# sdrobert/pydrobert-pytorch

Measured on AMD Instinct MI355X. Metric: utterances/sec (N=4096,T=512) error_rate+ctc_beam at 1/2/4/8 GPU, higher is better.
Workload: dtype f32

## Files before the change

### pydrobert-pytorch_amd/csrc/ctc_frame.hpp

```cpp
#pragma once
#include "wave_select.hpp"

namespace pdt {

#ifdef PDT_STAMPS
__device__ unsigned long long g_stamps[16];
__device__ unsigned long long *g_stamp_lds_dummy;
#define PDT_STAMP(ph)                                                        \
  do {                                                                       \
    const unsigned long long now_ = __builtin_readcyclecounter();           \
    pdt_stamp_acc[ph] += (unsigned)(now_ - stamp_last_);                     \
    stamp_last_ = now_;                                                      \
  } while (0)
#define PDT_STAMP_BEGIN unsigned long long stamp_last_ = __builtin_readcyclecounter()
#else
#define PDT_STAMP(ph) do {} while (0)
#define PDT_STAMP_BEGIN do {} while (0)
#endif

#ifdef PDT_STATS
__device__ unsigned long long g_stats[24];
#define PDT_STAT(i) do { if (lane_id() == 0) atomicAdd(&g_stats[i], 1ull); } while (0)
#else
#define PDT_STAT(i) do {} while (0)
#endif

#ifdef PDT_UTT_STATS
__device__ unsigned g_utt_stats[8192 * 4];
#define PDT_UTT(k, v) do { pdt_utt_acc[k] += (unsigned)(v); } while (0)
#else
#define PDT_UTT(k, v) do {} while (0)
#endif

constexpr int kMaxWidth = 32;

struct CtcArgs {
  const float *logits;
  int64_t lg_st, lg_sn, lg_sv;
  const int64_t *lens;
  int T, N, V, W, S;
  int64_t *y;
  int64_t *y_lens;
  float *y_probs;
  int2 *trie;
  int2 *ckpt;
  unsigned char *grow;
  int ckpt_shift, ckpt_count;
  int lds_per_wave, waves_per_wg;
  int exact_div;
  int no_lean_extra;
  int no_steady;
};

struct Beam {
  float nb, b;
  int last, len, node;
  unsigned isp;
  int origin = 0;
};

__device__ __forceinline__ u64 readlane_u64(u64 v, int l) {
  const unsigned lo = (unsigned)__builtin_amdgcn_readlane((int)(unsigned)v, l);
  const unsigned hi = (unsigned)__builtin_amdgcn_readlane((int)(unsigned)(v >> 32), l);
  return ((u64)hi << 32) | lo;
}
__device__ __forceinline__ float readlane_f(float v, int l) {
  return __int_as_float(__builtin_amdgcn_readlane(__float_as_int(v), l));
}
__device__ __forceinline__ float shfl_f(float v, int l) { return __int_as_float(shfl_i(__float_as_int(v), l)); }
__device__ __forceinline__ unsigned fresh_zero() {
  unsigned z;
  asm volatile("v_mov_b32 %0, 0" : "=v"(z));
  return z;
}

struct DenseCtx {
  const float *ext;
  int64_t ext_sk, ext_sv;
  const int64_t *y_prev;
  int64_t yp_ss, yp_sk;
  int S;
  int lists_ready;
  const float *etab = nullptr;
  int etab_stride = 0;
  const int16_t *y_prev16 = nullptr;
  const int *slot = nullptr;
  const int *list_id = nullptr;
  unsigned closed = 0u;
  const int *lpos = nullptr;
  int lpos_stride = 0;
};

__host__ __device__ inline int nxt_stride(int W) { return W * W < 128 ? 128 : W * W; }
__host__ __device__ inline int consumer_scratch_bytes(int W) {
  return (2 * nxt_stride(W) * 4 + (W > 0 ? W : 1) * 4 * 3 + 7) & ~7;
}

struct FrameLds {
  u64 *surv;
  int *tl_tok;
  float *tl_p;
  unsigned char *pos;
  unsigned *chm;
  int *info;
  int *nxt_old, *nxt_new;
  int list_len;
  float *hdr;
  int2 *trie_u = nullptr;
  float pl_in = 0.0f, pblank_in = 0.0f;
  static __host__ __device__ size_t bytes(int V, int W, int Kp, bool dense) {
    const int RS = W > Kp ? W : Kp;
    size_t b = (size_t)PDT_SURV_CAP * 8 + (size_t)(dense ? Kp : 1) * PDT_WAVE * 8;
    b += dense ? 0 : (size_t)((V + 15) & ~15);
    b += (size_t)RS * 4 + (size_t)2 * W * 4 + (dense ? 0 : (size_t)2 * W * W * 4);
    return (b + 15) & ~(size_t)15;
  }
  __device__ void carve(unsigned char *base, int V, int W, int Kp, bool dense) {
    const int RS = W > Kp ? W : Kp, L = dense ? Kp : 1;
    surv = reinterpret_cast<u64 *>(base);
    tl_tok = reinterpret_cast<int *>(surv + PDT_SURV_CAP);
    tl_p = reinterpret_cast<float *>(tl_tok + L * PDT_WAVE);
    chm = reinterpret_cast<unsigned *>(tl_p + L * PDT_WAVE);
    info = reinterpret_cast<int *>(chm + RS);
    nxt_old = info + 2 * W;
    nxt_new = nxt_old + (dense ? 0 : W * W);
    pos = reinterpret_cast<unsigned char *>(nxt_new + (dense ? 0 : W * W));
  }
};

__device__ __forceinline__ int ctc_list_len(int V, int W, int Kp) {
  const int K = min(W, Kp * (V + 1));
  return min(V, K + Kp);
}

template <bool LONG = false>
__device__ __forceinline__ void build_shared_list(const float *p, float inv, int V, int M, u64 *surv,
                                                  int *tl_tok, float *tl_p, unsigned char *pos,
                                                  const unsigned *lmax_in = nullptr,
                                                  unsigned *probe = nullptr, int probe_rank = 1) {
  const int lane = lane_id();
  const u64 tk = wave_top_sorted<LONG, true>(p, V, M, surv, lmax_in, probe, probe_rank);
  if (lane < M) {
    const int tok = (int)idx_of(tk);
    tl_tok[lane] = tok;
    tl_p[lane] = p[tok] * inv;
    pos[tok] = (unsigned char)lane;
  }
}

#if defined(PDT_STAMPS)
#define PDT_STAMP_PARAM , unsigned *pdt_stamp_acc
#define PDT_STAMP_ARG , pdt_stamp_acc
#elif defined(PDT_UTT_STATS)
#define PDT_STAMP_PARAM , unsigned *pdt_utt_acc
#define PDT_STAMP_ARG , pdt_utt_acc
#else
#define PDT_STAMP_PARAM
#define PDT_STAMP_ARG
#endif

template <bool DENSE, bool ROWLESS = false, bool TRIE = !DENSE>
__device__ __forceinline__ bool ctc_frame(Beam &bm, const float *p, const float inv, const int V,
                                          const int W, const int Kp, const int t,
                                          const int64_t n, const CtcArgs &a, const DenseCtx &dc,
                                          const FrameLds &L, int &new_src, int &new_tok,
                                          int &new_kind PDT_STAMP_PARAM) {
  int lane = lane_id();
  asm volatile("" : "+v"(lane));
  const bool live = lane < Kp;
  const int K = min(W, Kp * (V + 1));
  const int M = min(V, K + Kp);
  const int me = live ? lane : 0;
  PDT_STAMP_BEGIN;

  if (DENSE && !dc.lists_ready) {
    for (int k = 0; k < Kp; ++k) {
      const u64 tk = wave_top_sorted_strided<true>(dc.ext + k * dc.ext_sk, dc.ext_sv, V, M, L.surv);
      if (lane < M) {
        L.tl_tok[k * PDT_WAVE + lane] = (int)idx_of(tk);
        L.tl_p[k * PDT_WAVE + lane] = fkey_inv(key_of(tk));
      }
      wave_sync();
    }
  }
  PDT_STAMP(1);
  auto list_of = [&](const int k) -> int { return DENSE ? (dc.list_id ? dc.list_id[k] : k) : 0; };
  const int my_list = list_of(me);
  const int *mt = L.tl_tok + my_list * PDT_WAVE;

  static_assert(!(DENSE && ROWLESS), "the row-less form reads the shared list");
  const float p_blank = ROWLESS ? L.pblank_in : p[V] * inv;
  const int lastc = min(max(bm.last, 0), V - 1);
  const float pl = ROWLESS ? L.pl_in : p[lastc] * inv;
  const float e_last = DENSE ? (dc.etab ? dc.etab[my_list * dc.etab_stride + me] : dc.ext[me * dc.ext_sk + lastc * dc.ext_sv]) : pl;
  const float tot = bm.nb + bm.b;
  const float B = tot * p_blank;
  float NB = bm.nb * pl;
  const bool valid_beam = live && tot > -PDT_INF;
  wave_sync();

  const int c_list = (DENSE || ROWLESS) ? M : min(L.list_len, M);
  const bool full_list = DENSE || ROWLESS || c_list >= M;
  int jl = -1;
  u64 avail = 0ull;
  bool s1_open = valid_beam, s2_open = valid_beam;
// ... 472 lines not shown
  PDT_STAMP(3);
  const int srcl = new_kind >= 0 ? new_src : lane;
  float NB_s = NB, B_s = B;
  int last_s = lastc, len_s = bm.len, node_s = bm.node;
  unsigned isp_s = bm.isp;
  if (!steady_f) {
    NB_s = shfl_f(NB, srcl), B_s = shfl_f(B, srcl);
    last_s = shfl_i(lastc, srcl), len_s = shfl_i(bm.len, srcl), node_s = shfl_i(bm.node, srcl);
    isp_s = (unsigned)shfl_i((int)bm.isp, srcl);
  }
  const bool is_ext = new_kind == 0 || new_kind == 1;
  const bool is_valid = new_kind >= 0;
  Beam nw;
  nw.nb = !is_valid ? -PDT_INF : (is_ext ? new_mass : NB_s);
  nw.b = !is_valid ? -PDT_INF : (is_ext ? 0.0f : B_s);
  nw.last = !is_valid ? 0 : (is_ext ? new_tok : last_s);
  nw.len = !is_valid ? 0 : len_s + (is_ext ? 1 : 0);
  nw.node = !is_valid ? -1 : (is_ext ? t * W + lane : node_s);
  if (TRIE) nw.origin = steady_f ? bm.origin : shfl_i(bm.origin, srcl);
  if (TRIE && is_valid && is_ext)
    *reinterpret_cast<int2 *>(reinterpret_cast<char *>(L.trie_u) + (unsigned)(t * W + lane) * 8u) = make_int2(node_s, new_tok);

  PDT_STAMP(4);
  const int RS = W > Kp ? W : Kp;
  if (!steady_f) {
    if (lane < RS) L.chm[lane] = fresh_zero();
    wave_sync();
    if (is_valid) atomicOr(&L.chm[new_src], 1u << lane);
  }
  if (is_valid) {
    L.info[2 * lane] = new_tok;
    L.info[2 * lane + 1] = len_s | (new_src << 20) | ((is_ext ? 1 : 0) << 28);
  }
  wave_sync();
  PDT_STAMP(10);
  unsigned isp_new = 0u;
  bool need_walk = false;
  bool pairs_done = false;
#ifndef PDT_NO_PAIR_PREFIX
#ifndef PDT_PAIR_DENSE
#define PDT_PAIR_DENSE 8
#endif
  if (__builtin_expect(TRIE && W <= 16 && !a.no_lean_extra && __ballot(is_valid && __popc(isp_s) > PDT_PAIR_DENSE) != 0ull, 0)) {
    const int pa = lane & 15, pq = lane >> 4;
    const u64 vmask = __ballot(is_valid);
    const int a_tok = shfl_i(new_tok, pa);
    const int a_w = shfl_i(len_s | (new_src << 20) | ((is_ext ? 1 : 0) << 28) | ((is_valid ? 1 : 0) << 29), pa);
    const unsigned a_isp = (unsigned)shfl_i((int)isp_s, pa);
    const int a_len_s = a_w & 0xFFFFF, a_src = (a_w >> 20) & 0xFF;
    const bool a_ext = (a_w >> 28) & 1, a_valid = (a_w >> 29) & 1;
    const int a_len = a_len_s + (a_ext ? 1 : 0);
    unsigned bits = 0u, walks = 0u;
#pragma unroll
    for (int r = 0; r < 4; ++r) {
      const int b = 4 * r + pq;
      const int tok_b = L.info[2 * b], w1 = L.info[2 * b + 1];
      const int lenB = w1 & 0xFFFFF, src_b = (w1 >> 20) & 0xFF;
      const bool ext_b = (w1 >> 28) & 1;
      const int len_b = lenB + (ext_b ? 1 : 0);
      bool pref = a_valid && ((vmask >> b) & 1ull) && b != pa && ((a_isp >> src_b) & 1u) && !(a_len > len_b);
      int tok_at = -1;
      if (pref) tok_at = lenB > a_len_s ? L.nxt_old[a_src * W + src_b] : (ext_b ? tok_b : -1);
      pref = pref && !(a_ext && tok_at != a_tok);
      bool walk = false;
      if (pref && a_len < len_b) {
        int nx;
        if (!a_ext) {
          nx = tok_at;
        } else if (lenB == a_len_s + 1) {
          nx = tok_b;
        } else {
          nx = -(2 + b);
          walk = true;
        }
        L.nxt_new[pa * W + b] = nx;
      }
      const u64 m = __ballot(pref), wm = __ballot(walk);
      const unsigned lo = (unsigned)m >> pa, hi = (unsigned)(m >> 32) >> pa;
      bits |= ((lo & 1u) | ((lo >> 15) & 2u) | ((hi & 1u) << 2) | ((hi >> 13) & 8u)) << (4 * r);
      walks |= (unsigned)(wm | (wm >> 16) | (wm >> 32) | (wm >> 48));
    }
    if (is_valid) {
      isp_new = bits | (1u << lane);
      need_walk = (walks >> lane) & 1u;
    }
    pairs_done = true;
    wave_sync();
  }
#endif
  if (is_valid && !pairs_done) {
    unsigned cand = 0u;
    if (steady_f) cand = isp_s;
    else
      for (unsigned m = isp_s; m; m &= m - 1u) cand |= L.chm[__builtin_ctz(m)];
    cand &= ~(1u << lane);
    isp_new = 1u << lane;
    while (cand) {
      const int b = __builtin_ctz(cand);
      cand &= cand - 1u;
      const int tok_b = L.info[2 * b], w1 = L.info[2 * b + 1];
      const int lenB = w1 & 0xFFFFF, src_b = (w1 >> 20) & 0xFF;
      const bool ext_b = (w1 >> 28) & 1;
      const int len_b = lenB + (ext_b ? 1 : 0);
      if (nw.len > len_b) continue;
      int tok_at;
      if (lenB > len_s)
        tok_at = !TRIE ? (dc.y_prev16 ? (int)dc.y_prev16[(int64_t)len_s * dc.yp_ss + (dc.slot ? dc.slot[src_b] : src_b) * dc.yp_sk]
                                      : (int)dc.y_prev[(int64_t)len_s * dc.yp_ss + (dc.slot ? dc.slot[src_b] : src_b) * dc.yp_sk])
                       : L.nxt_old[new_src * W + src_b];
      else
        tok_at = ext_b ? tok_b : -1;
      if (is_ext && tok_at != new_tok) continue;
      isp_new |= 1u << b;
      if (TRIE && nw.len < len_b) {
        int nx;
        if (!is_ext) {
          nx = tok_at;
        } else if (lenB == len_s + 1) {
          nx = tok_b;
        } else {
          nx = -(2 + b);
          need_walk = true;
        }
        L.nxt_new[lane * W + b] = nx;
      }
    }
  }
  if (TRIE && __ballot(need_walk)) {
    __builtin_amdgcn_fence(__ATOMIC_RELEASE, "agent");
    for (int b = 0; b < K; ++b) {
      const int node_b = __builtin_amdgcn_readlane(node_s, b);
      const int lenB = __builtin_amdgcn_readlane(len_s, b);
      if (need_walk && ((isp_new >> b) & 1u) && L.nxt_new[lane * W + b] == -(2 + b)) {
        int node = node_b, depth = lenB, tok = -1;
        while (node >= 0) {
          const int2 *rec = a.trie + ((int64_t)n * a.T * W + node);
          const int par_ = __hip_atomic_load(&rec->x, __ATOMIC_RELAXED, __HIP_MEMORY_SCOPE_AGENT);
          tok = __hip_atomic_load(&rec->y, __ATOMIC_RELAXED, __HIP_MEMORY_SCOPE_AGENT);
          if (depth == nw.len + 1) break;
          node = par_;
          --depth;
        }
        L.nxt_new[lane * W + b] = tok;
      }
    }
  }
  nw.isp = isp_new;
  bm = nw;
  wave_sync();
  PDT_STAMP(5);
  return list_sufficed;
}

template <int JW = 4>
__device__ __forceinline__ void walk_trie_segments(const int2 *tab, const int nseg, const int W, const int2 *trie_u,
                                                   int64_t *y_n, const int64_t row_stride) {
  const int lane = lane_id();
  for (int base = 0; base < nseg; base += JW * PDT_WAVE) {
    int node[JW], ps[JW], stop[JW], col[JW];
#pragma unroll
    for (int j = 0; j < JW; ++j) {
      const int sg = base + j * PDT_WAVE + lane;
      node[j] = -1, ps[j] = -1, stop[j] = 0, col[j] = 0;
      if (sg < nseg) {
        const int c = sg / W;
        col[j] = sg - c * W;
        const int2 top = tab[sg];
        stop[j] = c > 0 ? tab[sg - W].y : 0;
        node[j] = top.x;
        ps[j] = top.y - 1;
      }
    }
    bool any = true;
    while (any) {
      any = false;
      u64 rec[JW];
      bool act[JW];
#pragma unroll
      for (int j = 0; j < JW; ++j) {
        act[j] = ps[j] >= stop[j] && node[j] >= 0;
        rec[j] = 0ull;
        if (act[j]) rec[j] = *reinterpret_cast<const u64 *>(trie_u + node[j]);
      }
#pragma unroll
      for (int j = 0; j < JW; ++j) {
        if (act[j]) {
          y_n[(int64_t)ps[j] * row_stride + col[j]] = (int64_t)(int)(unsigned)(rec[j] >> 32);
          node[j] = (int)(unsigned)rec[j];
          --ps[j];
          any = true;
        }
      }
    }
  }
}

}
```

### pydrobert-pytorch_amd/csrc/ctc_search.hip

```cpp
#include "ctc_ring.hpp"
#include "switches.hpp"

#include <cstdlib>

namespace pdt {

template <int P, int NT = -1, bool INREG = (P == 1), bool GROW = false, int WC = -1, int VC = -1, bool PAIR = false>
__global__ void __launch_bounds__(256, INREG ? 8 : 4)
ctc_search_kernel(const CtcArgs a, const RingLayout rl_arg) {
  static_assert(!INREG || P == 1, "the register-resident row pass is a one-producer form");
  static_assert((WC > 0 && VC > 0) ? (P == 1 && INREG && !GROW) : true, "compile-time shapes: the register-resident form");
  const RingLayout rl = (WC > 0 && VC > 0) ? ring_layout(VC, WC, PDT_RING_STAGES, PDT_UTT_PER_WG, 1) : rl_arg;
  static_assert(!GROW || !INREG, "rows in the workspace are a form of the generic row pass");
  static_assert(NT < 0 || INREG, "compile-time chunk counts belong to the register-resident row pass");
  extern __shared__ __align__(16) unsigned char smem[];
  const int lane = lane_id();
  const int wave = __builtin_amdgcn_readfirstlane((int)(threadIdx.x >> 6));
  const int u = wave / (P + 1);
  const int role = wave - u * (P + 1);
  const bool producer = role < P;
  const int64_t n_raw = (int64_t)xcd_remap(blockIdx.x, gridDim.x) * rl.utt_per_wg + u;
  const bool idle = u >= rl.utt_per_wg || n_raw >= a.N;
  const int64_t n = idle ? 0 : n_raw;
  const int V = VC > 0 ? VC : a.V, W = WC > 0 ? WC : a.W;
// ... 299 lines not shown
#pragma unroll
          for (int i = 0; i < kPrefetch; ++i) {
            if (i > nt) break;
            if (i < nt) {
              pre[i] = nrow[(int64_t)(i * PDT_WAVE) * lg_sv];
            } else if (i == nt) {
              if (in_row) pre[i] = nrow[(int64_t)(i * PDT_WAVE) * lg_sv];
            }
          }
        }
      } else {
        float mx = -PDT_INF;
#pragma unroll
        for (int i = 0; i < kPrefetch; ++i) {
          const int v = lane + i * PDT_WAVE;
          if (v <= V) {
            p[v] = pre[i];
            mx = fmaxf(mx, pre[i]);
          }
        }
        {
          const float *row = a.logits + (int64_t)t * a.lg_st + n * lg_sn;
          int v = lane + kPrefetch * PDT_WAVE;
          if constexpr (!INREG) {
            for (; v + (kBatch - 1) * PDT_WAVE <= V; v += kBatch * PDT_WAVE) {
              float x[kBatch];
#pragma unroll
              for (int i = 0; i < kBatch; ++i) x[i] = row[(int64_t)(v + i * PDT_WAVE) * lg_sv];
#pragma unroll
              for (int i = 0; i < kBatch; ++i) {
                p[v + i * PDT_WAVE] = x[i];
                mx = fmaxf(mx, x[i]);
              }
            }
            for (; v <= V; v += 8 * PDT_WAVE) {
              float x[8];
#pragma unroll
              for (int i = 0; i < 8; ++i)
                x[i] = v + i * PDT_WAVE <= V ? row[(int64_t)(v + i * PDT_WAVE) * lg_sv] : -PDT_INF;
#pragma unroll
              for (int i = 0; i < 8; ++i) {
                if (v + i * PDT_WAVE <= V) p[v + i * PDT_WAVE] = x[i];
                mx = fmaxf(mx, x[i]);
              }
            }
          }
          for (; v <= V; v += PDT_WAVE) {
            const float x = row[(int64_t)v * lg_sv];
            p[v] = x;
            mx = fmaxf(mx, x);
          }
        }
        if (t + P < Tn) {
          const float *nrow = a.logits + (int64_t)(t + P) * a.lg_st + n * lg_sn + (int64_t)lane * lg_sv;
#pragma unroll
          for (int i = 0; i < kPrefetch; ++i) {
            const int v = lane + i * PDT_WAVE;
            if (v <= V) pre[i] = nrow[(int64_t)(i * PDT_WAVE) * lg_sv];
          }
        }
        mx = wave_max_f(mx);
        {
          int v = lane;
          if constexpr (!INREG) {
            for (; v + 7 * PDT_WAVE <= V; v += 8 * PDT_WAVE) {
              float x[8];
#pragma unroll
              for (int i = 0; i < 8; ++i) x[i] = p[v + i * PDT_WAVE];
#pragma unroll
              for (int i = 0; i < 8; ++i) {
                const float e = exp_nonpos(x[i] - mx);
                p[v + i * PDT_WAVE] = e;
                s += e;
              }
            }
          }
          for (; v <= V; v += PDT_WAVE) {
            const float e = exp_nonpos(p[v] - mx);
            p[v] = e;
            s += e;
          }
        }
      }
      s = wave_sum_f(s);
      wave_sync();
      const int M = ctc_list_len(V, W, (t == 0 && !(WC > 0 && VC > 0 && VC + 1 >= WC)) ? 1 : W);
      const float inv0 = __builtin_amdgcn_rcpf(s);
      float inv = __builtin_fmaf(__builtin_fmaf(-s, inv0, 1.0f), inv0, inv0);
      if (VC <= 0 && a.exact_div) {
        for (int v = lane; v <= V; v += PDT_WAVE) p[v] = p[v] / s;
        wave_sync();
        inv = 1.0f;
      }
      int Ml = M;
      if (short_ok && nshort >= kShortMin && nshort <= kShortMax) {
        PDT_STAT(1);
        const unsigned sk = lane < nshort ? surv32[lane] : 0u;
        unsigned st = nshort <= 16 ? row_sort_desc<unsigned>(sk) : half_wave_sort_desc<unsigned>(sk);
        const unsigned st_next = (unsigned)__builtin_amdgcn_mov_dpp((int)st, 0x130, 0xf, 0xf, true);
        int tok = 511 - (int)(st & 511u);
        if (__ballot(lane + 1 < nshort && (st >> 9) == (st_next >> 9)) != 0ull) {
          const int tk0 = 511 - (int)((lane < nshort ? surv32[lane] : 0u) & 511u);
          const u64 tk = half_wave_sort_desc<u64>(lane < nshort ? pack_key(fkey_nonneg(p[tk0]), (unsigned)tk0) : 0ull);
          tok = (int)idx_of(tk);
        }
        Ml = min(nshort, M);
        if (lane < Ml) {
          tl_tok[lane] = tok;
          slot_p(sl)[lane] = p[tok] * inv;
          pos[tok] = (unsigned char)lane;
        }
        const float step = fmaxf(fabsf(thr_off) * 0.03125f, 1e-3f);
        thr_off += nshort > kShortHi ? step : (nshort < kShortLo ? -step : 0.0f);
      } else {
        PDT_STAT(nshort > kShortMax ? 3 : 2);
        unsigned probe = 0u;
        build_shared_list<!INREG>(p, inv, V, M, surv, tl_tok, slot_p(sl), pos, INREG ? &lmax : nullptr,
                                  &probe, kProbeRank);
        if (short_ok) thr_off = mx_of_row + __logf(fkey_nonneg_inv(probe)) - mean;
      }
      PDT_STAT(0);
      if (lane == 0) {
        hdr[0] = inv;
        hdr[2] = __int_as_float(Ml);
      }
      wave_sync();
      if (lane == 0)
        __hip_atomic_store(&ready[P == 1 ? 0 : sl], t + 1, __ATOMIC_RELEASE, __HIP_MEMORY_SCOPE_WORKGROUP);
    }
    return;
  }

#ifndef PDT_NO_PRIO
  __builtin_amdgcn_s_setprio(PDT_CONSUMER_PRIO);
#endif
  FrameLds L;
  L.surv = surv;
  L.trie_u = a.trie + (int64_t)n * a.T * W;
  L.nxt_old = reinterpret_cast<int *>(cs);
  L.nxt_new = L.nxt_old + nxt_stride(W);
  L.chm = reinterpret_cast<unsigned *>(L.nxt_new + nxt_stride(W));
  L.info = reinterpret_cast<int *>(L.chm + W);
  Beam bm;
  bm.nb = lane == 0 ? 0.0f : -PDT_INF;
  bm.b = lane == 0 ? 1.0f : -PDT_INF;
  bm.last = 0;
  bm.len = 0;
  bm.node = -1;
  bm.isp = lane == 0 ? 1u : 0u;
  bm.origin = lane;
  constexpr bool kFullFromStart = WC > 0 && VC > 0 && VC + 1 >= WC;
  int Kp = kFullFromStart ? WC : 1;
  int fail_score = 0, full_mode = 0;
  const int ckpt_shift = (WC > 0 && VC > 0) ? 5 : a.ckpt_shift;
#ifdef PDT_STAMPS
  unsigned pdt_stamp_acc[14] = {0};
#endif
  int sl = 0;
#ifdef PDT_UTT_STATS
  const unsigned long long utt_t0_ = __builtin_readcyclecounter();
  unsigned pdt_utt_acc[4] = {0, 0, 0, 0};
#endif
  for (int t = 0; t < Tn; ++t, sl = sl + 1 == NS ? 0 : sl + 1) {
    PDT_STAMP_BEGIN;
#ifdef PDT_UTT_STATS
    const unsigned long long w0_ = __builtin_readcyclecounter();
#endif
    if (__hip_atomic_load(&ready[P == 1 ? 0 : sl], __ATOMIC_ACQUIRE, __HIP_MEMORY_SCOPE_WORKGROUP) <= t) {
#ifndef PDT_NO_PRIO
      __builtin_amdgcn_s_setprio(0);
#endif
      do {
        __builtin_amdgcn_s_sleep(PDT_SPIN_SLEEP);
      } while (__hip_atomic_load(&ready[P == 1 ? 0 : sl], __ATOMIC_ACQUIRE, __HIP_MEMORY_SCOPE_WORKGROUP) <= t);
#ifndef PDT_NO_PRIO
      __builtin_amdgcn_s_setprio(PDT_CONSUMER_PRIO);
#endif
    }
    PDT_STAMP(0);
#if defined(PDT_UTT_STATS) && !defined(PDT_UTT_REASONS)
    PDT_UTT(3, (__builtin_readcyclecounter() - w0_) >> 4);
#endif
    L.tl_tok = slot_tok(sl);
    L.tl_p = slot_p(sl);
    L.pos = slot_pos(sl);
    L.hdr = slot_hdr(sl);
    L.list_len = __float_as_int(slot_hdr(sl)[2]);
    const float s = slot_hdr(sl)[0];
    int ns, nt, nk;
    int lane_t = lane;
#ifndef PDT_SKIP_CONSUMER
    bool enough = true;
    if (!(readlane_f(bm.nb + bm.b, 0) == 0.0f)) {
      enough = ctc_frame<false>(bm, slot_row(sl), s, V, W, Kp, t, n, a, DenseCtx{}, L, ns, nt, nk PDT_STAMP_ARG);
      int *tmp = L.nxt_old;
      L.nxt_old = L.nxt_new;
      L.nxt_new = tmp;
      if (!kFullFromStart) Kp = W;
    }
    const int enough_s = __builtin_amdgcn_readfirstlane(enough ? 1 : 0);
    fail_score = enough_s ? max(fail_score - 1, 0) : min(fail_score + 1, 32);
    const int wf = fail_score > 16 ? 1 : (fail_score < 4 ? 0 : full_mode);
    if (wf != full_mode) {
      full_mode = wf;
      asm volatile("" : "+v"(lane_t));
      if (lane_t == 0) __hip_atomic_store(want_full, wf, __ATOMIC_RELAXED, __HIP_MEMORY_SCOPE_WORKGROUP);
    }
#else
    ns = nt = nk = 0; (void)s;
    if (!kFullFromStart) Kp = W;
#endif
    asm volatile("" : "+v"(lane_t));
    if (lane_t == 0) __hip_atomic_store(consumed, t + 1, __ATOMIC_RELEASE, __HIP_MEMORY_SCOPE_WORKGROUP);
    if (((t + 1) & ((1 << ckpt_shift) - 1)) == 0) {
      const int c = ((t + 1) >> ckpt_shift) - 1;
      if (lane_t < W)
        a.ckpt[((int64_t)n * a.ckpt_count + c) * W + lane_t] = make_int2(bm.node, bm.len | (bm.origin << 24));
      bm.origin = lane_t;
    }
  }

#ifdef PDT_UTT_STATS
  if (lane == 0 && n < 8192) {
    g_utt_stats[n * 4 + 0] = (unsigned)((__builtin_readcyclecounter() - utt_t0_) >> 4);
    for (int k = 1; k < 4; ++k) g_utt_stats[n * 4 + k] = pdt_utt_acc[k];
  }
#endif
#ifdef PDT_STAMPS
  if (lane == 0)
    for (int i = 0; i < 14; ++i) atomicAdd(&g_stamps[i], (unsigned long long)pdt_stamp_acc[i]);
  unsigned long long stamp_last_ = __builtin_readcyclecounter();
#endif
  if (lane < W) {
    a.y_probs[n * W + lane] = bm.nb + bm.b;
    a.y_lens[n * W + lane] = bm.len;
  }
  __builtin_amdgcn_fence(__ATOMIC_RELEASE, "workgroup");
  __builtin_amdgcn_fence(__ATOMIC_ACQUIRE, "agent");
#ifndef PDT_SKIP_WALK
  {
    const int C = Tn >> ckpt_shift;
    int2 *tab = reinterpret_cast<int2 *>(ring);
    if (lane < W) {
      const bool ok = bm.node >= 0;
      tab[C * W + lane] = make_int2(bm.node, bm.len);
      int cur = bm.origin;
      for (int c = C - 1; c >= 0; --c) {
        const int2 rec = a.ckpt[((int64_t)n * a.ckpt_count + c) * W + cur];
        const int nd = rec.x, lo = rec.y;
        tab[c * W + lane] = ok ? make_int2(nd, lo & 0xFFFFFF) : make_int2(-1, 0);
        cur = lo >> 24;
      }
    }
    wave_sync();
#ifdef PDT_STAMPS
    unsigned long long st1_ = __builtin_readcyclecounter();
    if (lane == 0) atomicAdd(&g_stamps[11], st1_ - stamp_last_);
#endif
    walk_trie_segments(tab, (C + 1) * W, W, a.trie + (int64_t)n * a.T * W, a.y + n * W, (int64_t)a.N * W);
#ifdef PDT_STAMPS
    unsigned long long st2_ = __builtin_readcyclecounter();
    if (lane == 0) atomicAdd(&g_stamps[12], st2_ - st1_);
#endif
    int lmin = lane < W ? bm.len : 0x7fffffff;
    for (int off = 32; off > 0; off >>= 1) lmin = min(lmin, shfl_i(lmin, lane ^ off));
    for (int f = lmin * W + lane; f < a.S * W; f += PDT_WAVE) {
      const int pos = f / W, k = f - pos * W;
      if (pos >= tab[C * W + k].y) a.y[((int64_t)pos * a.N + n) * W + k] = 0;
    }
  }
#endif
#ifdef PDT_STAMPS
  if (lane == 0) atomicAdd(&g_stamps[6], __builtin_readcyclecounter() - stamp_last_);
#endif
}

template <int P, int NT = -1, bool INREG = (P == 1), bool GROW = false, int WC = -1, int VC = -1, bool PAIR = false>
static int launch_ctc_search_p(const CtcArgs &a, const RingLayout &rl, hipStream_t stream) {
  const size_t smem = (size_t)rl.utt_bytes * rl.utt_per_wg;
  if (const int rc = set_lds(ctc_search_kernel<P, NT, INREG, GROW, WC, VC, PAIR>, smem)) return rc;
  const unsigned grid = (unsigned)((a.N + rl.utt_per_wg - 1) / rl.utt_per_wg);
  hipLaunchKernelGGL((ctc_search_kernel<P, NT, INREG, GROW, WC, VC, PAIR>), dim3(grid), dim3(64 * (P + 1) * rl.utt_per_wg), smem,
                     stream, a, rl);
  return (int)hipGetLastError();
}

__host__ inline int ckpt_shift_for(int T, int W, const RingLayout &rl) {
  const size_t ring = (size_t)rl.slot_bytes * rl.nstage;
  int sh = 5;
  while (((size_t)(T >> sh) + 1) * W * sizeof(int2) > ring) ++sh;
  return sh;
}

struct CtcPlan {
  int producers, nstage, utt_per_wg, inreg;
};
__host__ inline int plan_ctc_search(int V, int W, CtcPlan *plan, RingLayout *rl) {
  if (W < 1 || W > kMaxWidth) return PDT_E_TOO_LONG;
  const size_t soft_cap = 64 * 1024, hard_cap = 160 * 1024;
  if (V + 1 > 8 * PDT_WAVE) {
    *rl = ring_layout(V, W, 4, 1, 3);
    if ((size_t)rl->utt_bytes * 4 <= hard_cap) return *plan = CtcPlan{3, 4, 1, 0}, PDT_OK;

    *rl = ring_layout(V, W, 3, 1, 3);
    if ((size_t)rl->utt_bytes <= hard_cap) return *plan = CtcPlan{3, 3, 1, 0}, PDT_OK;
    *rl = ring_layout(V, W, 4, 1, 3, true);
    return *plan = CtcPlan{3, 4, 1, 2}, PDT_OK;
  }
  int nstage = PDT_RING_STAGES, upw = PDT_UTT_PER_WG;
  *rl = ring_layout(V, W, nstage, upw, 1);
  while ((size_t)rl->utt_bytes * upw > soft_cap && (upw > 1 || nstage > 2)) {
    if (upw > 1) upw = 1; else nstage = 2;
    *rl = ring_layout(V, W, nstage, upw, 1);
  }
  if ((size_t)rl->utt_bytes * upw > hard_cap) return PDT_E_TOO_LONG;
  return *plan = CtcPlan{1, nstage, upw, 1}, PDT_OK;
}

bool ctc_rowreg_applies(int V, int W);
void ctc_rowreg_plan(int V, int W, int32_t *plan5);
int launch_ctc_rowreg(CtcArgs a, hipStream_t stream);

int launch_ctc_search(const CtcArgs &a, const CtcPlan &plan, const RingLayout &rl, hipStream_t stream) {
  if (plan.inreg == 2) return launch_ctc_search_p<3, -1, false, true>(a, rl, stream);
  if (plan.producers == 3) return launch_ctc_search_p<3>(a, rl, stream);
#ifndef PDT_NO_V256
  {
    const RingLayout c = ring_layout(256, 16, PDT_RING_STAGES, PDT_UTT_PER_WG, 1);
    if (a.V == 256 && a.W == 16 && a.ckpt_shift == 5 && !a.exact_div && !a.no_lean_extra && a.lg_sv == 1 && a.lg_sn == 257 && c.nstage == rl.nstage && c.utt_per_wg == rl.utt_per_wg && c.utt_bytes == rl.utt_bytes &&
        c.slot_bytes == rl.slot_bytes) {
      if (switches().ctc_pair != 0 && rl.nstage == 4) return launch_ctc_search_p<1, 4, true, false, 16, 256, true>(a, rl, stream);
      return launch_ctc_search_p<1, 4, true, false, 16, 256>(a, rl, stream);
    }
  }
#endif
#ifndef PDT_NO_WIDTH16
  if (a.V / PDT_WAVE == 4 && a.W == 16) return launch_ctc_search_p<1, 4, true, false, 16>(a, rl, stream);
#endif
  if (a.V / PDT_WAVE == 4) return launch_ctc_search_p<1, 4>(a, rl, stream);
  return launch_ctc_search_p<1>(a, rl, stream);
}

}

extern "C" {

static int64_t ctc_trie_bytes(int64_t T, int64_t N, int64_t width) {
  return ((T + T / 32 + 1) * N * width * (int64_t)sizeof(int2) + 255) & ~(int64_t)255;
}

int64_t pdt_ctc_prefix_search_workspace_bytes(int64_t T, int64_t N, int64_t V, int64_t width) {
  if (T < 0 || N < 0 || V < 1 || width < 1 || V >= (1 << 30)) return 0;
  int64_t bytes = ctc_trie_bytes(T, N, width) + 16;
  pdt::CtcPlan plan;
  pdt::RingLayout rl;
  if (pdt::plan_ctc_search((int)V, (int)(width > pdt::kMaxWidth ? pdt::kMaxWidth : width), &plan, &rl) == PDT_OK &&
      rl.row_global)
    bytes += N * (int64_t)rl.nstage * rl.g_slot_bytes;
  return bytes;
}

int pdt_ctc_prefix_search_plan(int64_t V, int64_t width, int32_t *plan5) {
  int32_t *plan4 = plan5;
  if (V < 1 || width < 1 || !plan5) return PDT_E_ARG;
  if (V >= (1 << 30)) return PDT_E_TOO_LONG;
  pdt::CtcPlan plan;
  pdt::RingLayout rl;
  const int rc = pdt::plan_ctc_search((int)V, (int)width, &plan, &rl);
  if (rc != PDT_OK) return rc;
  plan4[0] = plan.producers; plan4[1] = plan.nstage; plan4[2] = plan.utt_per_wg; plan4[3] = plan.inreg;
  plan5[4] = 0;
  if (pdt::ctc_rowreg_applies((int)V, (int)width)) pdt::ctc_rowreg_plan((int)V, (int)width, plan5);
  return PDT_OK;
}

int pdt_ctc_prefix_search(const float *logits, int64_t T, int64_t N, int64_t V, int64_t lg_st,
                          int64_t lg_sn, int64_t lg_sv, const int64_t *lens, int64_t width,
                          int64_t S, int64_t *y, int64_t *y_lens, float *y_probs,
                          void *workspace, void *stream) {
  using namespace pdt;
  if (T < 0 || N < 0 || V < 1 || width < 1 || S < 0) return PDT_E_ARG;
  if (N == 0) return PDT_OK;
  if (!y_lens || !y_probs || (T > 0 && (!logits || !workspace)) || (S > 0 && !y)) return PDT_E_ARG;
  if (width > kMaxWidth) return PDT_E_TOO_LONG;
  if (T * width >= (1ll << 31) || V >= (1 << 30) || N >= (1ll << 31) || T >= (1 << 24)) return PDT_E_TOO_LONG;
  CtcArgs a{};
  a.logits = logits; a.lg_st = lg_st; a.lg_sn = lg_sn; a.lg_sv = lg_sv;
  a.lens = lens;
  a.T = (int)T; a.N = (int)N; a.V = (int)V; a.W = (int)width; a.S = (int)S;
  a.y = y; a.y_lens = y_lens; a.y_probs = y_probs;
  a.trie = reinterpret_cast<int2 *>(workspace);
  a.ckpt = a.trie + T * N * width;
  a.grow = reinterpret_cast<unsigned char *>(workspace) + ctc_trie_bytes(T, N, width);
  a.exact_div = switches().ctc_exact_div == 1 ? 1 : 0;
  a.no_lean_extra = switches().ctc_lean_extra == 0 ? 1 : 0;
  a.no_steady = switches().ctc_steady == 0 ? 1 : 0;
  if (ctc_rowreg_applies(a.V, a.W) && lg_sv == 1) return launch_ctc_rowreg(a, (hipStream_t)stream);
  CtcPlan plan;
  RingLayout rl;
  const int rc = plan_ctc_search(a.V, a.W, &plan, &rl);
  if (rc != PDT_OK) return rc;
  a.ckpt_shift = ckpt_shift_for((int)T, (int)width, rl);
  a.ckpt_count = (int)(T >> a.ckpt_shift) + 1;
  return launch_ctc_search(a, plan, rl, (hipStream_t)stream);
}

}

#ifdef PDT_STATS
extern "C" int pdt_debug_read_stats(unsigned long long *host24, int reset) {
  hipError_t e = hipMemcpyFromSymbol(host24, HIP_SYMBOL(pdt::g_stats), sizeof(unsigned long long) * 24);
  if (e == hipSuccess && reset) {
    unsigned long long z[24] = {0};
    e = hipMemcpyToSymbol(HIP_SYMBOL(pdt::g_stats), z, sizeof(z));
  }
  return (int)e;
}
#endif

#ifdef PDT_UTT_STATS
extern "C" int pdt_debug_read_utt_stats(unsigned *host, int count, int reset) {
  hipError_t e = hipMemcpyFromSymbol(host, HIP_SYMBOL(pdt::g_utt_stats), sizeof(unsigned) * 4 * (size_t)count);
  if (e == hipSuccess && reset) {
    static unsigned z[8192 * 4];
    e = hipMemcpyToSymbol(HIP_SYMBOL(pdt::g_utt_stats), z, sizeof(z));
  }
  return (int)e;
}
#endif

#ifdef PDT_STAMPS
extern "C" int pdt_debug_read_stamps(unsigned long long *host16, int reset) {
  hipError_t e = hipMemcpyFromSymbol(host16, HIP_SYMBOL(pdt::g_stamps), sizeof(unsigned long long) * 16);
  if (e == hipSuccess && reset) {
    unsigned long long z[16] = {0};
    e = hipMemcpyToSymbol(HIP_SYMBOL(pdt::g_stamps), z, sizeof(z));
  }
  return (int)e;
}
#endif
```

### pydrobert-pytorch_amd/csrc/pdt_api.hip

```cpp
#include <cmath>
#include <algorithm>
#include <cstdlib>

#include "lev_launch.hpp"
#include "switches.hpp"
#include <cstring>
#include <mutex>

namespace pdt {
static bool costs_exact_in_f32(float ins, float del, float sub, int64_t R, int64_t H) {
  const float c[3] = {ins, del, sub};
  float mx = 0.0f;
  for (float v : c) {
    if (!std::isfinite(v)) return false;
    mx = std::fmax(mx, std::fabs(v));
  }
  for (int q = 0; q <= 20; ++q) {
    bool ok = true;
    for (float v : c) {
      const float s = std::ldexp(v, q);
      ok = ok && (s == std::floor(s));
    }
    if (ok) {
      const double bound = (double)(R + H + 2) * (double)std::ldexp(mx, q);
      return bound < 16777216.0;
    }
  }
  return false;
}

static bool bitpar_enabled() { return switches().lev_bitpar != 0; }

static bool oc_bitpar_enabled() { return switches().oc_bitpar != 0; }

namespace {
struct SwitchName {
  const char *name;
  int Switches::*field;
  int deft;
};
const SwitchName kSwitchNames[] = {
    {"PDT_LEV_BITPAR", &Switches::lev_bitpar, 1},         {"PDT_OC_BITPAR", &Switches::oc_bitpar, 1},
    {"PDT_CTC_EXACT_DIV", &Switches::ctc_exact_div, 0},   {"PDT_CTC_ROWREG", &Switches::ctc_rowreg, 1},
    {"PDT_STEP_WIDE", &Switches::step_wide, 0},           {"PDT_CTC_LEAN_EXTRA", &Switches::ctc_lean_extra, 1},
    {"PDT_CTC_PAIR", &Switches::ctc_pair, 1},             {"PDT_STEP_FLAT", &Switches::step_flat, 1},
    {"PDT_CTC_STEADY", &Switches::ctc_steady, 1},
};
}

Switches &switches() {
  static Switches s = [] {
    Switches v{};
    for (const SwitchName &n : kSwitchNames) {
      const char *e = std::getenv(n.name);
      v.*(n.field) = (e && e[0]) ? std::atoi(e) : n.deft;
    }
    return v;
  }();
  return s;
}

namespace {
std::mutex g_kept_mu;
const void *g_kept[16] = {};
unsigned g_kept_next = 0;
}
static void kept_tables_forget(const void *ws) {
  std::lock_guard<std::mutex> lock(g_kept_mu);
  for (const void *&e : g_kept)
    if (e == ws) e = nullptr;
}
static void kept_tables_note(const void *ws) {
  kept_tables_forget(ws);
  std::lock_guard<std::mutex> lock(g_kept_mu);
  g_kept[g_kept_next++ % 16] = ws;
}
static bool kept_tables_has(const void *ws) {
  std::lock_guard<std::mutex> lock(g_kept_mu);
  for (const void *e : g_kept)
    if (e == ws) return true;
  return false;
}

static int fill_common(LevArgs &a, const int64_t *ref, int64_t R, int64_t ref_st, int64_t ref_sn,
                       const int64_t *hyp, int64_t H, int64_t hyp_st, int64_t hyp_sn, int64_t N,
                       int has_eos, int64_t eos, int include_eos, float ins, float del, float sub) {
  if (R < 0 || H < 0 || N < 0) return PDT_E_ARG;
  if (N > 0 && ((R > 0 && !ref) || (H > 0 && !hyp))) return PDT_E_ARG;
  if (R > (1 << 28) || H > (1 << 28) || N > (1ll << 31) - 1) return PDT_E_TOO_LONG;
  a = LevArgs{};
  a.ref = ref; a.hyp = hyp;
  a.ref_st = ref_st; a.ref_sn = ref_sn; a.hyp_st = hyp_st; a.hyp_sn = hyp_sn;
  a.R = (int)R; a.H = (int)H; a.N = (int)N;
  a.has_eos = has_eos; a.eos = eos; a.include_eos = include_eos;
  a.ins = ins; a.del = del; a.sub = sub; a.mult = 1.0f;
  return PDT_OK;
}
}

extern "C" {

int pdt_amd_abi_version(void) { return 14; }

int pdt_amd_set_switch(const char *name, int value) {
  if (!name) return PDT_E_ARG;
  for (const pdt::SwitchName &n : pdt::kSwitchNames)
    if (std::strcmp(n.name, name) == 0) return pdt::switches().*(n.field) = value, PDT_OK;
  return PDT_E_ARG;
}

int pdt_amd_get_switch(const char *name, int *value) {
  if (!name || !value) return PDT_E_ARG;
  for (const pdt::SwitchName &n : pdt::kSwitchNames)
    if (std::strcmp(n.name, name) == 0) return *value = pdt::switches().*(n.field), PDT_OK;
  return PDT_E_ARG;
}

int64_t pdt_lev_workspace_bytes(int64_t R, int64_t H, int64_t N) {
  if (R < 0 || H < 0 || N <= 0) return 0;
  int64_t need = 0;
  if (pdt::bitpar_enabled()) {
    const pdt::BitparPlan p = pdt::plan_bitpar(H, R, N);
    if (p.ok) need = (int64_t)p.total;
  }
  if (R > 64 * 32) need = std::max(need, pdt::lev_workgroup_ws_per_utt(R, H, nullptr) * N);
  return need;
}

static int lev_entry(const int64_t *ref, int64_t R, int64_t ref_st, int64_t ref_sn, const int64_t *hyp,
                     int64_t H, int64_t hyp_st, int64_t hyp_sn, int64_t N, int has_eos, int64_t eos,
                     int include_eos, float ins_cost, float del_cost, float sub_cost, int norm, int mode,
                     int exclude_last, float padding, int return_mistakes, float *out, int64_t out_sh,
                     int64_t out_sn, int64_t *ref_lens_out, int64_t *hyp_lens_out, int32_t *status,
                     void *workspace, int64_t workspace_bytes, void *stream, pdt::LevTables tables) {
  using namespace pdt;
  if (mode != PDT_MODE_FINAL && mode != PDT_MODE_PREFIX) return PDT_E_ARG;
  if (exclude_last && mode != PDT_MODE_PREFIX) return PDT_E_ARG;
  if (exclude_last && H == 0) return PDT_E_ARG;
  if (N > 0 && !out) return PDT_E_ARG;
  float mult = 1.0f;
  if (ins_cost == del_cost && del_cost == sub_cost && sub_cost > 0.0f) {
    if (!return_mistakes) mult = ins_cost;
    ins_cost = del_cost = sub_cost = 1.0f;
    return_mistakes = 0;
  }
  LevArgs a;
  int rc = fill_common(a, ref, R, ref_st, ref_sn, hyp, H, hyp_st, hyp_sn, N, has_eos, eos,
                       include_eos, ins_cost, del_cost, sub_cost);
  if (rc != PDT_OK) return rc;
  if (N == 0) return PDT_OK;
  a.mult = mult;
  a.norm = norm; a.mode = mode; a.exclude_last = exclude_last; a.count = return_mistakes;
  a.padding = padding;
  a.out = out; a.out_sh = out_sh; a.out_sn = out_sn;
  a.ref_lens_out = ref_lens_out; a.hyp_lens_out = hyp_lens_out; a.status = status;
  if (!return_mistakes && !costs_exact_in_f32(ins_cost, del_cost, sub_cost, R, H)) {
    if (R > 64 * 32) return launch_lev_workgroup(a, true, workspace, workspace_bytes, (hipStream_t)stream);
    return launch_lev_rowsync(a, true, (hipStream_t)stream);
  }
  if (!return_mistakes && ins_cost == 1.0f && del_cost == 1.0f && sub_cost == 1.0f && workspace &&
      bitpar_enabled()) {
    const BitparPlan p = plan_bitpar(H, R, N);
    if (p.ok && (int64_t)p.total <= workspace_bytes) {
      if (tables == kTablesGiven && !kept_tables_has(workspace)) tables = kTablesOwn;
      rc = launch_lev_bitpar(a, p, workspace, (hipStream_t)stream, tables);
      if (tables == kTablesKeep || (tables == kTablesOwn && !p.fused)) kept_tables_note(workspace);
      else if (tables == kTablesOwn) kept_tables_forget(workspace);
      return rc;
    }
  }
  return launch_lev_skewed(a, (hipStream_t)stream);
}

int pdt_lev(const int64_t *ref, int64_t R, int64_t ref_st, int64_t ref_sn, const int64_t *hyp,
            int64_t H, int64_t hyp_st, int64_t hyp_sn, int64_t N, int has_eos, int64_t eos,
            int include_eos, float ins_cost, float del_cost, float sub_cost, int norm, int mode,
            int exclude_last, float padding, int return_mistakes, float *out, int64_t out_sh,
            int64_t out_sn, int64_t *ref_lens_out, int64_t *hyp_lens_out, int32_t *status,
            void *workspace, int64_t workspace_bytes, void *stream) {
  return lev_entry(ref, R, ref_st, ref_sn, hyp, H, hyp_st, hyp_sn, N, has_eos, eos, include_eos, ins_cost,
                   del_cost, sub_cost, norm, mode, exclude_last, padding, return_mistakes, out, out_sh, out_sn,
                   ref_lens_out, hyp_lens_out, status, workspace, workspace_bytes, stream, pdt::kTablesOwn);
}

int pdt_lev_keep(const int64_t *ref, int64_t R, int64_t ref_st, int64_t ref_sn, const int64_t *hyp,
                 int64_t H, int64_t hyp_st, int64_t hyp_sn, int64_t N, int has_eos, int64_t eos,
                 int include_eos, float ins_cost, float del_cost, float sub_cost, int norm, int mode,
                 int exclude_last, float padding, int return_mistakes, float *out, int64_t out_sh,
                 int64_t out_sn, int64_t *ref_lens_out, int64_t *hyp_lens_out, int32_t *status,
                 void *workspace, int64_t workspace_bytes, void *stream) {
  return lev_entry(ref, R, ref_st, ref_sn, hyp, H, hyp_st, hyp_sn, N, has_eos, eos, include_eos, ins_cost,
                   del_cost, sub_cost, norm, mode, exclude_last, padding, return_mistakes, out, out_sh, out_sn,
                   ref_lens_out, hyp_lens_out, status, workspace, workspace_bytes, stream, pdt::kTablesKeep);
}

int pdt_lev_classified(const int64_t *ref, int64_t R, int64_t ref_st, int64_t ref_sn, const int64_t *hyp,
                       int64_t H, int64_t hyp_st, int64_t hyp_sn, int64_t N, int has_eos, int64_t eos,
                       int include_eos, float ins_cost, float del_cost, float sub_cost, int norm, int mode,
                       int exclude_last, float padding, int return_mistakes, float *out, int64_t out_sh,
// ... 62 lines not shown
```

### pydrobert-pytorch_amd/csrc/switches.hpp

```cpp
#pragma once

namespace pdt {

struct Switches {
  int lev_bitpar;
  int oc_bitpar;
  int ctc_exact_div;
  int ctc_rowreg;
  int step_wide;
  int ctc_pair;
  int step_flat;
  int ctc_lean_extra;
  int ctc_steady;
};

Switches &switches();

}
```

### pydrobert-pytorch_amd/pydrobert_amd/switches.py

```python

import contextlib
import ctypes
import os

from . import _cabi

_HOST_DEFAULTS = {
    "PDT_LEV_CACHE": 0,
    "PDT_CTC_LM_FUSED": 1,
    "PDT_CTC_LM_TABLE": 1,
    "PDT_BEAM_FUSED": 1,
    "PDT_BEAM_SEARCH": 1,
    "PDT_BEAM_TABLE": 1,
    "PDT_CHECK_INVARIANTS": 0,
    "PDT_WALK_TABLE": 1,
}
_NATIVE = (
    "PDT_LEV_BITPAR", "PDT_OC_BITPAR", "PDT_CTC_EXACT_DIV", "PDT_CTC_ROWREG", "PDT_STEP_WIDE",
    "PDT_CTC_LEAN_EXTRA", "PDT_CTC_PAIR", "PDT_STEP_FLAT", "PDT_CTC_STEADY",
)


def _from_env(name, default):
    raw = os.environ.get(name, "")
    try:
        return int(raw) if raw != "" else default
    except ValueError:
        return default


_values = {name: _from_env(name, deft) for name, deft in _HOST_DEFAULTS.items()}


def names():
    return tuple(_HOST_DEFAULTS) + _NATIVE


def get(name: str) -> int:
    if name in _values:
        return _values[name]
    if name in _NATIVE:
        out = ctypes.c_int(0)
        _cabi.check(_cabi.lib().pdt_amd_get_switch(name.encode(), ctypes.addressof(out)), "pdt_amd_get_switch")
        return out.value
    raise KeyError(name)


def set(name: str, value: int) -> None:
    if name in _values:
        _values[name] = int(value)
    elif name in _NATIVE:
        _cabi.check(_cabi.lib().pdt_amd_set_switch(name.encode(), int(value)), "pdt_amd_set_switch")
    else:
        raise KeyError(name)


@contextlib.contextmanager
def override(**kw):
    old = {k: get(k) for k in kw}
    try:
        for k, v in kw.items():
            set(k, v)
        yield
    finally:
        for k, v in old.items():
            set(k, v)
```

Baseline: 2.159 million.

## Add in-place fast path for CTC beam frames when each beam extends uniquely

Adds ctc_frame_inplace, which checks with wave ballots and DPP max-reductions whether each of the K full beams has an unrelated, strictly ordered top extension that dominates every other candidate. When that holds, each beam is extended in place and its trie record written, skipping the full per-frame candidate selection. A decline counter gates the check so it only retries every few frames after repeated failures. The cost is extra ballot and reduction work on frames where the fast path does not apply. A new switch controls it, on by default.

After: 2.396 million, median of 6. 10.9% higher.

```diff
diff --git a/pydrobert-pytorch_amd/csrc/ctc_frame.hpp b/pydrobert-pytorch_amd/csrc/ctc_frame.hpp
--- a/pydrobert-pytorch_amd/csrc/ctc_frame.hpp
+++ b/pydrobert-pytorch_amd/csrc/ctc_frame.hpp
@@ -50,7 +50,17 @@
   int exact_div;
   int no_lean_extra;
   int no_steady;
+  int no_inplace;
 };
+
+#ifndef PDT_INPLACE_DECLINES
+#define PDT_INPLACE_DECLINES 4
+#endif
+#ifndef PDT_INPLACE_PERIOD
+#define PDT_INPLACE_PERIOD 16
+#endif
+constexpr int kInplaceDeclines = PDT_INPLACE_DECLINES, kInplacePeriod = PDT_INPLACE_PERIOD;
+static_assert((kInplacePeriod & (kInplacePeriod - 1)) == 0, "the period is a mask of the frame index");
 
 struct Beam {
   float nb, b;
@@ -829,6 +839,52 @@
   return list_sufficed;
 }
 
+__device__ __forceinline__ bool ctc_frame_inplace(Beam &bm, const float *p, const float inv, const int V,
+                                                  const int c_list, const int K, const int W, const int t,
+                                                  const FrameLds &L) {
+  int lane = lane_id();
+  asm volatile("" : "+v"(lane));
+  const float tot = bm.nb + bm.b;
+  const bool live = lane < K;
+  const unsigned first_k = (1u << K) - 1u;
+  const unsigned full = (unsigned)__ballot(live && tot > -PDT_INF) & first_k;
+  const u64 related = __ballot(live && (bm.isp & ~(1u << lane)) != 0u);
+  if (full != first_k || related != 0ull || c_list < 3) return false;
+  const int lastc = min(max(bm.last, 0), V - 1);
+  const unsigned q = L.pos[lastc];
+  const float p_blank = p[V] * inv, pl = p[lastc] * inv;
+  unsigned key0 = 0u, rest = 0u;
+  int tok = 0;
+  if (live) {
+    const int j0 = q == 0u ? 1 : 0, j1 = q <= 1u ? 2 : 1;
+    tok = L.tl_tok[j0];
+    key0 = fkey_nonneg(tot * L.tl_p[j0]);
+    const float NB = bm.nb * pl, B = tot * p_blank;
+    rest = max(max(fkey_nonneg(tot * L.tl_p[j1]), fkey_nonneg(bm.b * pl)), fkey_nonneg(NB + B));
+  }
+  const unsigned key_next = (unsigned)__builtin_amdgcn_mov_dpp((int)key0, 0x101, 0xf, 0xf, true);
+  const unsigned desc = (unsigned)__ballot(key0 >= key_next) & (first_k >> 1);
+  unsigned rmax = rest;
+  rmax = max(rmax, (unsigned)dpp_or<PDT_DPP_ROW_SHR(1)>((int)rmax, 0));
+  rmax = max(rmax, (unsigned)dpp_or<PDT_DPP_ROW_SHR(2)>((int)rmax, 0));
+  rmax = max(rmax, (unsigned)dpp_or<PDT_DPP_ROW_SHR(4), 0xf, 0xe>((int)rmax, 0));
+  rmax = max(rmax, (unsigned)dpp_or<PDT_DPP_ROW_SHR(8), 0xf, 0xc>((int)rmax, 0));
+  const unsigned others = (unsigned)__builtin_amdgcn_readlane((int)rmax, 15);
+  const unsigned kth = (unsigned)__builtin_amdgcn_readlane((int)key0, K - 1);
+  if (desc != (first_k >> 1) || !(kth > max(others, 64u))) return false;
+  PDT_STAT(17);
+  if (live) {
+    *reinterpret_cast<int2 *>(reinterpret_cast<char *>(L.trie_u) + (unsigned)(t * W + lane) * 8u) = make_int2(bm.node, tok);
+    bm.nb = fkey_nonneg_inv(key0);
+    bm.b = 0.0f;
+    bm.last = tok;
+    bm.len = bm.len + 1;
+    bm.node = t * W + lane;
+  }
+  wave_sync();
+  return true;
+}
+
 template <int JW = 4>
 __device__ __forceinline__ void walk_trie_segments(const int2 *tab, const int nseg, const int W, const int2 *trie_u,
                                                    int64_t *y_n, const int64_t row_stride) {
diff --git a/pydrobert-pytorch_amd/csrc/ctc_search.hip b/pydrobert-pytorch_amd/csrc/ctc_search.hip
--- a/pydrobert-pytorch_amd/csrc/ctc_search.hip
+++ b/pydrobert-pytorch_amd/csrc/ctc_search.hip
@@ -475,6 +475,7 @@
   constexpr bool kFullFromStart = WC > 0 && VC > 0 && VC + 1 >= WC;
   int Kp = kFullFromStart ? WC : 1;
   int fail_score = 0, full_mode = 0;
+  int inplace_gate = 0;
   const int ckpt_shift = (WC > 0 && VC > 0) ? 5 : a.ckpt_shift;
 #ifdef PDT_STAMPS
   unsigned pdt_stamp_acc[14] = {0};
@@ -515,7 +516,13 @@
 #ifndef PDT_SKIP_CONSUMER
     bool enough = true;
     if (!(readlane_f(bm.nb + bm.b, 0) == 0.0f)) {
-      enough = ctc_frame<false>(bm, slot_row(sl), s, V, W, Kp, t, n, a, DenseCtx{}, L, ns, nt, nk PDT_STAMP_ARG);
+      bool decided = false;
+      if (W <= 16 && Kp == W && V >= W && !a.no_inplace && (inplace_gate < kInplaceDeclines || (t & (kInplacePeriod - 1)) == 0)) {
+        decided = ctc_frame_inplace(bm, slot_row(sl), s, V, L.list_len, W, W, t, L);
+        const int decided_s = __builtin_amdgcn_readfirstlane(decided ? 1 : 0);
+        inplace_gate = decided_s ? 0 : min(inplace_gate + 1, kInplaceDeclines);
+      }
+      if (!decided) enough = ctc_frame<false>(bm, slot_row(sl), s, V, W, Kp, t, n, a, DenseCtx{}, L, ns, nt, nk PDT_STAMP_ARG);
       int *tmp = L.nxt_old;
       L.nxt_old = L.nxt_new;
       L.nxt_new = tmp;
@@ -718,6 +725,7 @@
   a.exact_div = switches().ctc_exact_div == 1 ? 1 : 0;
   a.no_lean_extra = switches().ctc_lean_extra == 0 ? 1 : 0;
   a.no_steady = switches().ctc_steady == 0 ? 1 : 0;
+  a.no_inplace = (switches().ctc_inplace == 0 || a.no_steady) ? 1 : 0;
   if (ctc_rowreg_applies(a.V, a.W) && lg_sv == 1) return launch_ctc_rowreg(a, (hipStream_t)stream);
   CtcPlan plan;
   RingLayout rl;
diff --git a/pydrobert-pytorch_amd/csrc/pdt_api.hip b/pydrobert-pytorch_amd/csrc/pdt_api.hip
--- a/pydrobert-pytorch_amd/csrc/pdt_api.hip
+++ b/pydrobert-pytorch_amd/csrc/pdt_api.hip
@@ -44,7 +44,7 @@
     {"PDT_CTC_EXACT_DIV", &Switches::ctc_exact_div, 0},   {"PDT_CTC_ROWREG", &Switches::ctc_rowreg, 1},
     {"PDT_STEP_WIDE", &Switches::step_wide, 0},           {"PDT_CTC_LEAN_EXTRA", &Switches::ctc_lean_extra, 1},
     {"PDT_CTC_PAIR", &Switches::ctc_pair, 1},             {"PDT_STEP_FLAT", &Switches::step_flat, 1},
-    {"PDT_CTC_STEADY", &Switches::ctc_steady, 1},
+    {"PDT_CTC_STEADY", &Switches::ctc_steady, 1},         {"PDT_CTC_INPLACE", &Switches::ctc_inplace, 1},
 };
 }
 
diff --git a/pydrobert-pytorch_amd/csrc/switches.hpp b/pydrobert-pytorch_amd/csrc/switches.hpp
--- a/pydrobert-pytorch_amd/csrc/switches.hpp
+++ b/pydrobert-pytorch_amd/csrc/switches.hpp
@@ -12,6 +12,7 @@
   int step_flat;
   int ctc_lean_extra;
   int ctc_steady;
+  int ctc_inplace;
 };
 
 Switches &switches();
diff --git a/pydrobert-pytorch_amd/pydrobert_amd/switches.py b/pydrobert-pytorch_amd/pydrobert_amd/switches.py
--- a/pydrobert-pytorch_amd/pydrobert_amd/switches.py
+++ b/pydrobert-pytorch_amd/pydrobert_amd/switches.py
@@ -18,6 +18,7 @@
 _NATIVE = (
     "PDT_LEV_BITPAR", "PDT_OC_BITPAR", "PDT_CTC_EXACT_DIV", "PDT_CTC_ROWREG", "PDT_STEP_WIDE",
     "PDT_CTC_LEAN_EXTRA", "PDT_CTC_PAIR", "PDT_STEP_FLAT", "PDT_CTC_STEADY",
+    "PDT_CTC_INPLACE",
 )
 
 
```
